# fzaiser/genfer

Hardware: AMD Instinct MI355X
Metric: TaylorPoly mul f64 GMAC/s (higher is better)
Workload: dtype f64

## Files before the change

genfer_amd/csrc/gft_conv_tiled.hip:

```cpp
#include <algorithm>
#include <cstdio>
#include <cstdlib>
#include <cstring>
#include <map>
#include <vector>

#include "gft_kernels.hpp"
#include "gft_peel_layout.hpp"

namespace gft {

namespace {

struct TileSeg {
    unsigned u, a, b;
    unsigned step_begin, step_end;
    int dest;
};

struct RedTile {
    unsigned u, a, b;
    unsigned first, count;
    unsigned slot0;
};

struct TiledArgs {
    unsigned xU, x0, x1, xI;
    unsigned yU, y0, y1, yI;
    unsigned zU, z0, z1, zI;
    unsigned nx8, ny8;
    unsigned nxc, nyc, nb;
    unsigned P1;
    unsigned tsh;
    unsigned slab_axis;
    unsigned slab_lo, slab_hi;
    int accumulate;
    unsigned xcd_remap;
    unsigned cut;
    unsigned lim1;
    size_t zsU, zs0, zs1, zoff;
    const double* xp;
    const double* yp;
    double* z;
    double* ws;
    const TileSeg* segs;
    const unsigned* wg_begin;
    const RedTile* red;
    const unsigned* red_slots;
    const unsigned* guard;
    unsigned guard_epoch;
    unsigned* claim;
    unsigned n_ranges, n_queues;
#ifdef GFT_TILED_DIAG
    unsigned long long* stamps;
#endif
    unsigned char blk1[8], blk2[8];
};

typedef const double __attribute__((address_space(4))) * cptr_t;

#ifndef GFT_TILED_DEFAULT_VARIANT
#define GFT_TILED_DEFAULT_VARIANT 7
#endif
#ifndef GFT_TILED_PEEL_DEFAULT
#define GFT_TILED_PEEL_DEFAULT -1
#endif
#ifndef GFT_TILED_PEEL_LANES_DEFAULT
#define GFT_TILED_PEEL_LANES_DEFAULT -1
#endif
constexpr unsigned PEEL_MIN_EXTENT = 112, PEEL_MIN_INNER = 64;

__device__ inline void loadx(double (&dst)[8], cptr_t p) {
#pragma unroll
    for (int i = 0; i < 8; ++i) dst[i] = p[i];
}

__device__ inline void load8(double (&dst)[8], const double* p) {
#pragma unroll
    for (int i = 0; i < 8; ++i) dst[i] = p[i];
}

__device__ inline void load8_b128(double (&dst)[8], const double* p) {
    const double2* q = reinterpret_cast<const double2*>(__builtin_assume_aligned(p, 16));
#pragma unroll
    for (int i = 0; i < 4; ++i) {
        double2 v = q[i];
        dst[2 * i] = v.x;
        dst[2 * i + 1] = v.y;
    }
}

// ... 351 lines not shown
                double* d = w + ((size_t)c1 * 64 + lane) * 8;
#pragma unroll
                for (int r = 0; r < 8; ++r) d[r] = acc1[r];
            }
            if (has2) {
                double* d = w + ((size_t)c2 * 64 + lane) * 8;
#pragma unroll
                for (int r = 0; r < 8; ++r) d[r] = acc2[r];
            }
        }
    }
#ifdef GFT_TILED_DIAG
    if (A.stamps && tid == 0) A.stamps[3 * (size_t)wg + 1] = __builtin_amdgcn_s_memrealtime();
#endif
    if (!claiming) break;
    }
}

__global__ void __launch_bounds__(256) k_conv_reduce(TiledArgs A, unsigned n_red) {
    const unsigned ti = blockIdx.x, c = blockIdx.y;
    if (ti >= n_red) return;
    if (A.guard && *A.guard == A.guard_epoch) return;
    __shared__ double part[3][64][8];
    const RedTile rt = A.red[ti];
    const unsigned lane = threadIdx.x & 63u, q = threadIdx.x >> 6;
    const unsigned k0 = (64u >> A.tsh) * rt.a + (lane >> A.tsh), k1 = (rt.b << A.tsh) + (lane & ((1u << A.tsh) - 1u));
    bool lane_in = k0 < A.z0 && k1 < A.z1;
    if (A.slab_axis == 1) lane_in = lane_in && k0 >= A.slab_lo && k0 < A.slab_hi;
    else if (A.slab_axis == 2) lane_in = lane_in && k1 >= A.slab_lo && k1 < A.slab_hi;
    double v[8];
#pragma unroll
    for (int r = 0; r < 8; ++r) v[r] = 0.0;
    double* zrow = A.z + A.zoff + (size_t)rt.u * A.zsU + (size_t)k0 * A.zs0 + (size_t)k1 * A.zs1;
    if (lane_in) {
        if (q == 0 && A.accumulate) {
#pragma unroll
            for (int r = 0; r < 8; ++r) {
                unsigned k2 = 8 * c + r;
                if (k2 < A.zI) v[r] = zrow[k2];
            }
        }
        const unsigned lo = (unsigned)((unsigned long long)rt.count * q / 4), hi = (unsigned)((unsigned long long)rt.count * (q + 1) / 4);
        unsigned p = lo;
        if (!A.red_slots) {
            const size_t stride = (size_t)A.nb * 512;
            const double* w = A.ws + (size_t)(rt.slot0 + lo) * stride + ((size_t)c * 64 + lane) * 8;
            for (; p + 4 <= hi; p += 4, w += 4 * stride) {
                double t[4][8];
#pragma unroll
                for (int u = 0; u < 4; ++u)
#pragma unroll
                    for (int r = 0; r < 8; ++r) t[u][r] = w[(size_t)u * stride + r];
#pragma unroll
                for (int u = 0; u < 4; ++u)
#pragma unroll
                    for (int r = 0; r < 8; ++r) v[r] += t[u][r];
            }
        }
        for (; p < hi; ++p) {
            const unsigned slot = A.red_slots ? A.red_slots[rt.first + p] : rt.slot0 + p;
            const double* w = A.ws + (size_t)slot * A.nb * 512 + ((size_t)c * 64 + lane) * 8;
#pragma unroll
            for (int r = 0; r < 8; ++r) v[r] += w[r];
        }
        if (q > 0) {
#pragma unroll
            for (int r = 0; r < 8; ++r) part[q - 1][lane][r] = v[r];
        }
    }
    __syncthreads();
    if (q == 0 && lane_in) {
#pragma unroll
        for (int g = 0; g < 3; ++g)
#pragma unroll
            for (int r = 0; r < 8; ++r) v[r] += part[g][lane][r];
#pragma unroll
        for (int r = 0; r < 8; ++r) {
            unsigned k2 = 8 * c + r;
            if (k2 < A.zI) zrow[k2] = v[r];
        }
    }
}

__global__ void __launch_bounds__(256) k_prep_operands(const double* __restrict__ x, double* __restrict__ xp, size_t x_rows,
                                                       unsigned xlen, unsigned nx8, const double* __restrict__ y,
                                                       double* __restrict__ yp, size_t y_rows, unsigned ylen, unsigned ny8,
                                                       unsigned* flag, unsigned epoch) {
    const size_t tx = x_rows * nx8, ty = yp ? y_rows * ny8 : y_rows * ylen;
    bool bad = false;
    for (size_t i = blockIdx.x * (size_t)blockDim.x + threadIdx.x; i < tx + ty; i += (size_t)gridDim.x * blockDim.x) {
        double v;
        if (i < tx) {
            size_t row = i / nx8;
            unsigned col = (unsigned)(i - row * nx8);
            v = col < xlen ? x[row * xlen + col] : 0.0;
            xp[i] = v;
        } else if (yp) {
            size_t k = i - tx, row = k / ny8;
            unsigned col = (unsigned)(k - row * ny8);
            v = col < ylen ? y[row * ylen + col] : 0.0;
            yp[k] = v;
        } else {
            v = y[i - tx];
        }
        if (!((v - v) == 0.0)) bad = true;
    }
    if (__any(bad) && (threadIdx.x & 63) == 0) atomicMax(flag, epoch);
}

__global__ void __launch_bounds__(256) k_pack_peel(const double* __restrict__ x, const double* __restrict__ y,
                                                   double* __restrict__ w0, double* __restrict__ s1, double* __restrict__ w1,
                                                   unsigned n0, unsigned n1, unsigned nI, unsigned n8) {
    const size_t t0 = (size_t)7 * (n0 / 8) * n1 * n8, ts = (size_t)7 * n0 * n8, t1 = (size_t)7 * (n1 / 8) * n0 * n8;
    for (size_t i = blockIdx.x * (size_t)blockDim.x + threadIdx.x; i < t0 + ts + t1; i += (size_t)gridDim.x * blockDim.x) {
        const double* src;
        double* dst;
        size_t row;
        unsigned col;
        if (i < t0) {
            row = i / n8;
            col = (unsigned)(i - row * n8);
            const unsigned r1 = (unsigned)(row % n1), va = (unsigned)(row / n1), a = va % (n0 / 8), v = va / (n0 / 8);
            src = x + ((size_t)(8 * a + 1 + v) * n1 + r1) * nI;
            dst = w0 + i;
        } else if (i < t0 + ts) {
            const size_t k = i - t0;
            row = k / n8;
            col = (unsigned)(k - row * n8);
            const unsigned j1c = (unsigned)(row % n0), ju = (unsigned)(row / n0);
            src = y + ((size_t)j1c * n1 + ju) * nI;
            dst = s1 + k;
        } else {
            const size_t k = i - t0 - ts;
            row = k / n8;
            col = (unsigned)(k - row * n8);
            const unsigned r = (unsigned)(row % n0), vb = (unsigned)(row / n0), b = vb % (n1 / 8), v = vb / (n1 / 8);
            src = x + ((size_t)r * n1 + 8 * b + 1 + v) * nI;
            dst = w1 + k;
        }
        *dst = col < nI ? src[col] : 0.0;
    }
}

__global__ void __launch_bounds__(256) k_pad_rows(const double* __restrict__ in, double* __restrict__ out, size_t rows,
                                                  unsigned len, unsigned P, unsigned B) {
    const size_t per_p = rows * B, total = per_p * P;
    for (size_t i = blockIdx.x * (size_t)blockDim.x + threadIdx.x; i < total; i += (size_t)gridDim.x * blockDim.x) {
        const unsigned p = (unsigned)(i / per_p);
        const size_t rem = i - (size_t)p * per_p, row = rem / B;
        const unsigned col = p * B + (unsigned)(rem - row * B);
        out[i] = col < len ? in[row * len + col] : 0.0;
    }
}
__global__ void __launch_bounds__(256) k_fold_rows(const double* __restrict__ zt, double* __restrict__ z, size_t rows,
                                                   size_t row_lo, size_t row_hi, unsigned Pz, unsigned B, unsigned zI,
                                                   int accumulate, const unsigned* guard, unsigned epoch) {
    if (guard && *guard == epoch) return;
    const unsigned RI = 2 * B - 1;
    size_t total = (row_hi - row_lo) * zI;
    for (size_t i = blockIdx.x * (size_t)blockDim.x + threadIdx.x; i < total; i += (size_t)gridDim.x * blockDim.x) {
        size_t row = row_lo + i / zI;
        unsigned k = (unsigned)(i % zI), p = k / B, r = k - p * B;
        double v = p < Pz ? zt[((size_t)p * rows + row) * RI + r] : 0.0;
        if (p > 0 && p - 1 < Pz && r + 1 < B) v += zt[((size_t)(p - 1) * rows + row) * RI + B + r];
        double* dst = z + row * zI + k;
        *dst = accumulate ? *dst + v : v;
    }
}


struct Variant {
    bool fast;
    bool b128;
    bool xcd;
    bool compact;
    bool peel;
    unsigned other;
};
static_assert((GFT_TILED_DEFAULT_VARIANT & 3) == 3, "only the pipelined b128 kernel (VAR 3) is instantiated for every NW");
Variant decode_variant(int variant, bool compact_operands) {
    if (variant < 0) variant = GFT_TILED_DEFAULT_VARIANT;
    Variant V = {bool(variant & 1), bool(variant & 2), bool(variant & 4), bool(variant & 8), bool(variant & 128),
                 unsigned(variant & ~(1 | 2 | 4 | 8 | 128))};
    if (compact_operands && V.fast && V.b128) V = {true, true, V.xcd, true, false, 0};
    else if (compact_operands) V.fast = V.b128 = false;
    return V;
}
int pick_var(const Variant& V, unsigned NW) {
    if (V.peel) return 131;
    if (V.compact) return 11;
    if (V.fast == V.b128 && !V.other) return V.fast ? 3 : 0;
    return (NW == 8 && V.fast && !V.b128 && !V.xcd) ? 1 + (int)V.other : -1;
}

struct PlanKey {
    unsigned v[19];
    bool operator<(const PlanKey& o) const { return std::memcmp(v, o.v, sizeof(v)) < 0; }
};

struct Plan {
    TiledArgs base;
    unsigned n_wg = 0, n_red = 0, n_slots = 0, NW = 0;
    unsigned n_resident = 0;
    unsigned n_segs = 0;
    bool all_slabs = false;
    size_t lds_bytes = 0;
    void* d_tables = nullptr;
};

struct TableArena {
    char* dev = nullptr;
    char* host = nullptr;
    size_t bytes = 0, head = 0;
    bool tried = false;
    bool ensure() {
        if (dev) return true;
        if (tried) return false;
        tried = true;
        const size_t n = 32u << 20;
        if (hipMalloc((void**)&dev, n) != hipSuccess) { dev = nullptr; (void)hipGetLastError(); return false; }
        if (hipHostMalloc((void**)&host, n, hipHostMallocDefault) != hipSuccess) {
            (void)hipFree(dev);
            dev = nullptr;
            (void)hipGetLastError();
// ... 345 lines not shown
    else GFT_LAUNCH((k_conv_tiled<NW, VAR | 256, TSH>), dim3(grid), dim3(NW * 64), P.lds_bytes, st, T);
}
template <int NW, int VAR>
void launch_main_nw(hipStream_t st, const Plan& P, const TiledArgs& T, unsigned grid) {
    if (T.tsh == 3) launch_main_t<NW, VAR, 3>(st, P, T, grid);
    else launch_main_t<NW, VAR, 0>(st, P, T, grid);
}
template <int VAR>
void launch_main(hipStream_t st, const Plan& P, const TiledArgs& T, unsigned grid) {
    switch (P.NW) {
        case 1: launch_main_nw<1, VAR>(st, P, T, grid); break;
        case 2: launch_main_nw<2, VAR>(st, P, T, grid); break;
        case 4: launch_main_nw<4, VAR>(st, P, T, grid); break;
        default: launch_main_nw<8, VAR>(st, P, T, grid); break;
    }
}

}

void tiled_pad_rows_f64(hipStream_t st, const double* in, double* out, size_t rows, unsigned len, unsigned P, unsigned B) {
    size_t tot = rows * P * B;
    if (!tot) return;
    GFT_LAUNCH(k_pad_rows, dim3((unsigned)std::min<size_t>((tot + 255) / 256, 4096)), dim3(256), 0, st, in, out, rows,
                       len, P, B);
}
void tiled_fold_rows_f64(hipStream_t st, const double* zt, double* z, size_t rows, size_t row_lo, size_t row_hi, unsigned Pz,
                         unsigned B, unsigned zI, int accumulate, const unsigned* guard, unsigned epoch) {
    size_t tot = (row_hi - row_lo) * zI;
    if (!tot) return;
    GFT_LAUNCH(k_fold_rows, dim3((unsigned)std::min<size_t>((tot + 255) / 256, 4096)), dim3(256), 0, st, zt, z, rows,
                       row_lo, row_hi, Pz, B, zI, accumulate, guard, epoch);
}

void tiled_set_lane_tile(int tsh) { tiled_force_tsh() = tsh; }
void tiled_set_slots(int n) { tiled_slots_cap() = n; }
void tiled_set_taper(int pct) { tiled_taper_pct() = pct < 0 ? GFT_TILED_TAPER_DEFAULT : std::min(pct, 90); }

namespace {

int& tiled_peel_mode() {
    static int v = GFT_TILED_PEEL_DEFAULT;
    return v;
}
int& tiled_peel_lanes_mode() {
    static int v = GFT_TILED_PEEL_LANES_DEFAULT;
    return v;
}

const Plan* cached_plan(const ConvArgs& a, const Variant& V, const PeelSpec& ps, hipStream_t st) {
    PlanKey key;
    std::memset(&key, 0, sizeof(key));
    if (a.nd < 2 || a.nd > 4) return nullptr;
    key.v[0] = (unsigned)a.nd | ((unsigned)a.slab_axis << 8) | ((unsigned)tiled_force_tsh() << 16) | ((unsigned)tiled_taper_pct() << 24);
    for (int i = 0; i < a.nd; ++i) {
        key.v[1 + i] = a.xs[i];
        key.v[5 + i] = a.ys[i];
        key.v[9 + i] = a.zs[i];
    }
    key.v[13] = a.slab_lo;
    key.v[14] = a.slab_hi;
    key.v[15] = (unsigned)a.accumulate;
    key.v[16] = (unsigned)(a.j0_min | (a.j0_excl << 8) | (a.j0_desc << 16));
    key.v[17] = V.b128;
    key.v[18] = ps.role | (ps.cut << 4) | (ps.lim1 << 8) | (ps.all_slabs << 12);
    auto& cache = plan_cache();
    auto it = cache.find(key);
    if (it == cache.end()) {
        Plan P;
        if (cache.size() >= 1024) reset_plan_cache(st);
        if (!build_plan(a, V, ps, P, st)) return nullptr;
        it = cache.emplace(key, P).first;
    }
    return &it->second;
}

unsigned launch_grid(const Plan& P) {
    if (tiled_slots_cap() < 0) return P.n_wg;
    unsigned g = std::min(P.n_wg, P.n_resident);
    if (tiled_slots_cap() > 0) g = std::min(g, (unsigned)tiled_slots_cap());
    return g;
}
bool plan_claims(const Plan& P) { return launch_grid(P) < P.n_wg; }
constexpr size_t CLAIM_BYTES = 256;
unsigned* claim_words(char* wb, unsigned launch) { return (unsigned*)wb + 8 * launch; }
void zero_claim_words(hipStream_t st, char* wb) {
    enqueue_task([=] { lq_note((hipMemsetAsync)(wb, 0, CLAIM_BYTES, st), nullptr, "hipMemsetAsync"); });
}

#ifdef GFT_TILED_DIAG
constexpr unsigned STAMP_RANGES = 65536;
unsigned long long* stamp_area(unsigned launch, const Plan& first) {
    static unsigned long long* d_stamps = nullptr;
    const char* stamps_min = std::getenv("GFT_TILED_STAMPS_MIN");
    if (!std::getenv("GFT_TILED_STAMPS") || first.n_wg < (stamps_min ? (unsigned)std::atoi(stamps_min) : 1024u)) return nullptr;
    if (!d_stamps && hipMalloc((void**)&d_stamps, 3 * (size_t)3 * STAMP_RANGES * sizeof(unsigned long long)) != hipSuccess) d_stamps = nullptr;
    return d_stamps ? d_stamps + (size_t)launch * 3 * STAMP_RANGES : nullptr;
}
struct StampedLaunch {
    const char* name;
    const unsigned long long* d_stamps;
    unsigned n, grid;
    bool claiming;
};
void dump_stamps(hipStream_t st, const StampedLaunch* ls, unsigned n_launches) {
    if (hipStreamSynchronize(st) != hipSuccess) return;
    FILE* f = std::fopen(std::getenv("GFT_TILED_STAMPS"), "a");
    if (!f) return;
    unsigned long long first_end = 0;
    for (unsigned l = 0; l < n_launches; ++l) {
        const unsigned n = ls[l].n;
        std::vector<unsigned long long> h(3 * (size_t)n);
        if (!ls[l].d_stamps || hipMemcpy(h.data(), ls[l].d_stamps, h.size() * 8, hipMemcpyDeviceToHost) != hipSuccess) continue;
        unsigned long long t0 = ~0ull, t1 = 0, last[8] = {0}, busy[8] = {0};
        unsigned cnt[8] = {0};
        for (unsigned r = 0; r < n; ++r) {
            const unsigned long long b = h[3 * (size_t)r], e = h[3 * (size_t)r + 1];
            const unsigned x = (unsigned)h[3 * (size_t)r + 2] & 7u;
            t0 = std::min(t0, b);
            t1 = std::max(t1, e);
            last[x] = std::max(last[x], e);
            busy[x] += e - b;
            cnt[x]++;
        }
        std::fprintf(f, "launch %s: %u ranges on %u workgroups (%s), %.1f us from first start to last end\n", ls[l].name, n, ls[l].grid,
                     ls[l].claiming ? "claiming" : "one range each", (t1 - t0) / 100.0);
        if (l == 0) first_end = t1;
        else
            std::fprintf(f, "  first range starts %+.1f us, last range ends %+.1f us relative to the last range end of launch %s\n",
                         ((double)t0 - (double)first_end) / 100.0, ((double)t1 - (double)first_end) / 100.0, ls[0].name);
        for (int x = 0; x < 8; ++x)
            std::fprintf(f, "  xcd %d: %5u ranges, range time %10.1f us in all, last range ends %8.1f us before the launch's last\n", x, cnt[x],
                         busy[x] / 100.0, (t1 - last[x]) / 100.0);
    }
    std::fclose(f);
}
#endif

bool launch_plan_main(hipStream_t st, const Plan& P, TiledArgs& T, const Variant& V, unsigned* claim) {
    const unsigned grid = launch_grid(P);
    const bool eighths = V.xcd && P.n_wg % 8 == 0;
    T.n_ranges = P.n_wg;
    if (grid < P.n_wg) {
        if (!claim) return false;
        T.claim = claim;
        T.n_queues = eighths ? 8u : 1u;
        T.xcd_remap = 0;
    } else {
        T.claim = nullptr;
        T.n_queues = 1;
        T.xcd_remap = eighths ? 1u : 0u;
    }
#ifdef GFT_TILED_DIAG
    if (P.n_wg > STAMP_RANGES) T.stamps = nullptr;
#endif
    switch (pick_var(V, P.NW)) {
        case 131: launch_main<131>(st, P, T, grid); break;
        case 11: launch_main<11>(st, P, T, grid); break;
        case 3: launch_main<3>(st, P, T, grid); break;
        case 0: launch_main<0>(st, P, T, grid); break;
        case 1: launch_main_nw<8, 1>(st, P, T, grid); break;
#ifdef GFT_TILED_DIAG
        case 17: launch_main_nw<8, 17>(st, P, T, grid); break;
        case 33: launch_main_nw<8, 33>(st, P, T, grid); break;
        case 49: launch_main_nw<8, 49>(st, P, T, grid); break;
        case 65: launch_main_nw<8, 65>(st, P, T, grid); break;
        case 113: launch_main_nw<8, 113>(st, P, T, grid); break;
#endif
        default: return false;
    }
    return true;
}
void launch_plan_reduce(hipStream_t st, const Plan& P, const TiledArgs& T) {
    if (P.n_red) {
        GFT_LAUNCH(k_conv_reduce, dim3(P.n_red, T.nb), dim3(256), 0, st, T, P.n_red);
    }
}
bool launch_plan(hipStream_t st, const Plan& P, TiledArgs T, const Variant& V, unsigned* claim) {
#ifdef GFT_TILED_DIAG
    T.stamps = stamp_area(0, P);
#endif
    if (!launch_plan_main(st, P, T, V, claim)) return false;
#ifdef GFT_TILED_DIAG
    if (T.stamps) {
        const StampedLaunch l = {"plain", T.stamps, P.n_wg, launch_grid(P), plan_claims(P)};
        dump_stamps(st, &l, 1);
    }
#endif
    launch_plan_reduce(st, P, T);
    return true;
}

struct Operands {
    bool inplace, pack_y;
    size_t o_ws, o_xp, o_yp, end;
};
Operands operand_layout(const TiledArgs& B, size_t n_slots, bool claims, const double* x, const double* y, int operands_slack) {
    auto al = [](size_t v) { return (v + 255) / 256 * 256; };
    const size_t x_rows = (size_t)B.xU * B.x0 * B.x1, y_rows = (size_t)B.yU * B.y0 * B.y1;
    Operands o;
    o.inplace = operands_slack && B.nx8 == B.xI && B.ny8 == B.yI && B.nxc >= B.nb && B.nyc >= B.nb && !((uintptr_t)y & 15) &&
                !((uintptr_t)x & 7);
    o.pack_y = !o.inplace && (B.ny8 != B.yI || ((uintptr_t)y & 15));
    o.o_ws = claims ? CLAIM_BYTES : 0;
    o.o_xp = o.o_ws + al(n_slots * B.nb * 512 * sizeof(double));
    o.o_yp = o.o_xp + al((x_rows * B.nx8 + 8) * sizeof(double));
    o.end = o.o_yp + al(y_rows * B.ny8 * sizeof(double));
    return o;
}
void bind_operands(hipStream_t st, const Operands& o, const double* x, const double* y, char* wb, unsigned* nf_flag,
                   unsigned nf_epoch, TiledArgs& T) {
    T.ws = (double*)(wb + o.o_ws);
    if (o.inplace) {
        T.xp = x;
        T.yp = y;
        T.guard = nullptr;
        T.guard_epoch = 0;
        return;
    }
    const size_t x_rows = (size_t)T.xU * T.x0 * T.x1, y_rows = (size_t)T.yU * T.y0 * T.y1;
    double *xp = (double*)(wb + o.o_xp), *yp = (double*)(wb + o.o_yp);
    const size_t tot = x_rows * T.nx8 + (o.pack_y ? y_rows * T.ny8 : y_rows * T.yI);
    GFT_LAUNCH(k_prep_operands, dim3((unsigned)std::min<size_t>((tot + 255) / 256, 2048)), dim3(256), 0, st, x, xp, x_rows, T.xI,
               T.nx8, y, o.pack_y ? yp : nullptr, y_rows, T.yI, T.ny8, nf_flag, nf_epoch);
    T.xp = xp;
    T.yp = o.pack_y ? yp : y;
    T.guard = nf_flag;
    T.guard_epoch = nf_epoch;
}

bool peel_applies(const ConvArgs& a, const Variant& V) {
    const int mode = tiled_peel_mode();
    if (mode == 0) return false;
    if (a.nd != 3 || a.slab_axis != 0 || a.slab_lo != 0 || a.slab_hi != a.zs[0]) return false;
    if (a.j0_min || a.j0_excl || a.j0_desc) return false;
    for (int i = 0; i < 3; ++i)
        if (a.xs[i] != a.zs[i] || a.ys[i] != a.zs[i]) return false;
    const unsigned n0 = a.zs[0], n1 = a.zs[1];
    if (n0 % 8 || n1 % 8 || n0 < 16 || n1 < 16 || a.zs[2] > 128) return false;
    if (!V.fast || !V.b128 || V.compact || V.peel || V.other) return false;
    TiledArgs T;
    std::memset(&T, 0, sizeof(T));
    T.x0 = T.y0 = T.z0 = n0;
    T.x1 = T.y1 = T.z1 = n1;
    if (pick_lane_tile(T) != 3) return false;
    return mode == 1 || (n0 >= PEEL_MIN_EXTENT && n1 >= PEEL_MIN_EXTENT && a.zs[2] >= PEEL_MIN_INNER);
}

int conv_tiled_peel(hipStream_t st, const double* x, const double* y, double* z, const ConvArgs& a, const Variant& V, void* ws,
                    size_t ws_bytes, size_t* ws_needed, unsigned* nf_flag, unsigned nf_epoch, bool* guarded, bool* forked) {
    const unsigned n0 = a.zs[0], n1 = a.zs[1], nI = a.zs[2];
    ConvArgs l0, l1;
    std::memset(&l0, 0, sizeof(l0));
    l0.nd = 4;
    l0.slab_lo = 0;
    l0.slab_hi = 7;
    l0.accumulate = 1;
    l1 = l0;
    Variant VL = V;
    VL.peel = true;
    const unsigned s0x[4] = {7, 1, n1, nI}, s0y[4] = {7, n0 / 8, n1, nI}, s1x[4] = {7, 1, n0, nI}, s1y[4] = {7, n1 / 8, n0, nI};
    for (int i = 0; i < 4; ++i) {
        l0.xs[i] = s0x[i]; l0.ys[i] = l0.zs[i] = s0y[i];
        l1.xs[i] = s1x[i]; l1.ys[i] = l1.zs[i] = s1y[i];
    }
    const int lanes_mode = tiled_peel_lanes_mode();
    bool can_fork = lanes_mode != 0 && stream_lanes().ok;
    if (can_fork) {
        hipStreamCaptureStatus cs = hipStreamCaptureStatusNone;
        if (hipStreamIsCapturing(st, &cs) != hipSuccess) (void)hipGetLastError();
        if (cs != hipStreamCaptureStatusNone) can_fork = false;
    }
    bool fork = can_fork && lanes_mode > 0;
    PeelSpec pm, p0, p1;
    pm.role = 1; pm.cut = 3;
    p0.role = 2; p0.zsU = (size_t)n1 * nI; p0.zs0 = 8 * p0.zsU; p0.zs1 = nI; p0.zoff = p0.zsU;
    p1.role = 3; p1.lim1 = 1; p1.zsU = nI; p1.zs0 = 8 * (size_t)nI; p1.zs1 = (size_t)n1 * nI; p1.zoff = nI;
    Plan PM, P0, P1;
    for (int attempt = 0;; ++attempt) {
        const unsigned long long gen = plan_generation();
        const Plan* q = cached_plan(a, V, pm, st);
        if (!q) return -1;
        PM = *q;
        for (int pass = 0; pass < 2; ++pass) {
            p0.all_slabs = p1.all_slabs = fork ? 1u : 0u;
            if (!(q = cached_plan(l0, VL, p0, st))) return -1;
            P0 = *q;
            if (!(q = cached_plan(l1, VL, p1, st))) return -1;
            P1 = *q;
            if (fork || !can_fork || !(plan_claims(P0) && plan_claims(P1))) break;
            fork = true;
        }
        if (gen == plan_generation()) break;
        if (attempt) return -1;
    }
    const TiledArgs& B = PM.base;
    if (B.tsh != 3) return -1;
    const bool claims = plan_claims(PM) || plan_claims(P0) || plan_claims(P1);
    Operands o = operand_layout(B, 0, claims, x, y, a.operands_slack);
    const size_t slots[3] = {PM.n_slots, P0.n_segs, P1.n_segs};
    const PeelLayout L = peel_layout_for(slots, n0, n1, B.nx8, claims);
    o.o_ws = L.o_slab[0];
    o.o_xp = L.o_xp;
    o.o_yp = L.o_yp;
    if (ws && ws_bytes < L.need) return -1;
    if (ws_needed) *ws_needed = L.need;
    if (guarded) *guarded = !o.inplace;
    if (!ws) return 1;

    const hipStream_t st0 = fork ? stream_lanes().st[0] : st, st1 = fork ? stream_lanes().st[1] : st;
    if (forked) *forked = fork;

    char* wb = (char*)ws;
    double *w0 = (double*)(wb + L.o_w0), *s1 = (double*)(wb + L.o_s1), *w1 = (double*)(wb + L.o_w1);
    TiledArgs T = B;
    if (claims) zero_claim_words(st, wb + L.o_claim);
    bind_operands(st, o, x, y, wb, nf_flag, nf_epoch, T);
    {
        const size_t tot = L.b_w0 / sizeof(double) + (L.b_s1 / sizeof(double) - 8) + L.b_w1 / sizeof(double);
        GFT_LAUNCH(k_pack_peel, dim3((unsigned)std::min<size_t>((tot + 255) / 256, 4096)), dim3(256), 0, st, x, y, w0, s1, w1, n0, n1,
                   nI, B.nx8);
    }
    if (fork) lanes_fork(st);
    T.z = z;
    TiledArgs T0 = P0.base, T1 = P1.base;
    T0.ws = (double*)(wb + L.o_slab[1]);
    T1.ws = (double*)(wb + L.o_slab[2]);
    T0.z = T1.z = z;
    T0.guard = T1.guard = T.guard;
    T0.guard_epoch = T1.guard_epoch = T.guard_epoch;
    T0.xp = T.yp;
    T0.yp = w0;
    T1.xp = s1;
    T1.yp = w1;
#ifdef GFT_TILED_DIAG
    T.stamps = stamp_area(0, PM);
    T0.stamps = stamp_area(1, PM);
    T1.stamps = stamp_area(2, PM);
#endif
    unsigned *const c = claim_words(wb + L.o_claim, 0), *const c0 = claim_words(wb + L.o_claim, 1), *const c1 = claim_words(wb + L.o_claim, 2);
    if (fork) {
        const bool ok = launch_plan_main(st, PM, T, V, c) && launch_plan_main(st0, P0, T0, VL, c0) && launch_plan_main(st1, P1, T1, VL, c1);
        if (ok) launch_plan_reduce(st, PM, T);
        lanes_join(st);
        if (!ok) return 0;
        launch_plan_reduce(st, P0, T0);
        launch_plan_reduce(st, P1, T1);
    } else {
        if (!launch_plan_main(st, PM, T, V, c)) return 0;
        launch_plan_reduce(st, PM, T);
        if (!launch_plan_main(st, P0, T0, VL, c0)) return 0;
        launch_plan_reduce(st, P0, T0);
        if (!launch_plan_main(st, P1, T1, VL, c1)) return 0;
        launch_plan_reduce(st, P1, T1);
    }
#ifdef GFT_TILED_DIAG
    if (T.stamps) {
        const StampedLaunch ls[3] = {{"M", T.stamps, PM.n_wg, launch_grid(PM), plan_claims(PM)},
                                     {"L0", T0.stamps, P0.n_wg, launch_grid(P0), plan_claims(P0)},
                                     {"L1", T1.stamps, P1.n_wg, launch_grid(P1), plan_claims(P1)}};
        dump_stamps(st, ls, 3);
    }
#endif
    return 1;
}

}

void tiled_set_peel(int mode) { tiled_peel_mode() = mode < 0 ? -1 : (mode ? 1 : 0); }
void tiled_set_peel_lanes(int mode) { tiled_peel_lanes_mode() = mode < 0 ? GFT_TILED_PEEL_LANES_DEFAULT : (mode ? 1 : 0); }

bool conv_tiled_f64(hipStream_t st, const double* x, const double* y, double* z, const ConvArgs& a, void* ws, size_t ws_bytes,
                    size_t* ws_needed, unsigned* nf_flag, unsigned nf_epoch, bool* guarded, bool* peeled, bool* forked) {
    bool compact_operands = false;
    if (a.nd >= 2 && a.nd <= 4) {
        const unsigned nb = (a.zs[a.nd - 1] + 7) / 8;
        compact_operands = (a.xs[a.nd - 1] + 7) / 8 < nb || (a.ys[a.nd - 1] + 7) / 8 < nb;
    }
    const Variant V = decode_variant(a.variant, compact_operands);
    if (peeled) *peeled = false;
    if (forked) *forked = false;
    if (peel_applies(a, V)) {
        const int r = conv_tiled_peel(st, x, y, z, a, V, ws, ws_bytes, ws_needed, nf_flag, nf_epoch, guarded, forked);
        if (r >= 0) {
            if (peeled) *peeled = r == 1;
            return r == 1;
        }
    }
    const Plan* P = cached_plan(a, V, PeelSpec(), st);
    if (!P) return false;
    const bool claims = plan_claims(*P);
    const Operands o = operand_layout(P->base, P->n_slots, claims, x, y, a.operands_slack);
    const size_t need = o.end + 256;
    if (guarded) *guarded = !o.inplace;
    if (ws_needed) *ws_needed = need;
    if (!ws) return true;
    if (ws_bytes < need) return false;
    TiledArgs T = P->base;
    if (claims) zero_claim_words(st, (char*)ws);
    bind_operands(st, o, x, y, (char*)ws, nf_flag, nf_epoch, T);
    T.z = z;
    return launch_plan(st, *P, T, V, claim_words((char*)ws, 0));
}

}
```

genfer_amd/csrc/gft_kernels.hip:

```cpp
#include "gft_kernels.hpp"
#include "gft_kernels_int.hpp"

#include <algorithm>
#include <chrono>
#include <condition_variable>
#include <cstring>
#include <mutex>
#include <stdexcept>
#include <string>
#include <thread>

namespace gft {

unsigned long long g_launches = 0;
unsigned long long g_host_horner_stats[16] = {0};
bool g_host_horner_runs = true;
int g_host_simd = -1;
unsigned long long g_launches_in_place = 0;
unsigned long long g_stream_ops = 0;

namespace {
constexpr uint64_t LQ_SLOTS = 1024;
struct LaunchQueue {
    std::atomic<uint64_t> head{0};
// ... 128 lines not shown
            msg += std::string(" launching ") + (name ? name : "a kernel");
        } else if (g_lq_err_what) {
            msg += std::string(" in queued ") + g_lq_err_what;
        }
        msg += " (issued by the launch thread; results computed since are invalid)";
        g_lq_err_set.store(false, std::memory_order_relaxed);
    }
    throw std::runtime_error(msg);
}

bool lq_enabled() { return g_lq.enabled; }
void lq_configure(int device, bool enabled) {
    g_lq.drain();
    g_lq.device = device;
    g_lq.enabled = enabled;
}
void lq_shutdown() {
    g_lq.shutdown();
    g_lq.report();
    g_lq_err_set.store(false);
}
void lq_report() {
    g_lq.drain();
    g_lq.report();
}
void launch_drain_nothrow() { g_lq.drain(); }
void launch_drain() {
    g_lq.drain();
    lq_raise();
}
LaunchSlot* lq_begin() {
    if (!g_lq.worker.joinable()) g_lq.start();
    const uint64_t t = g_lq.tail.load(std::memory_order_relaxed);
    if (g_lq.trace && t - g_lq.head.load(std::memory_order_acquire) >= LQ_SLOTS) {
        const auto t0 = std::chrono::steady_clock::now();
        while (t - g_lq.head.load(std::memory_order_acquire) >= LQ_SLOTS) __builtin_ia32_pause();
        g_lq.tr_full_ns += LaunchQueue::ns_since(t0);
        g_lq.tr_full_n++;
    }
    while (t - g_lq.head.load(std::memory_order_acquire) >= LQ_SLOTS) __builtin_ia32_pause();
    return &g_lq.slots[t & (LQ_SLOTS - 1)];
}
void lq_commit() {
    g_lq.tail.store(g_lq.tail.load(std::memory_order_relaxed) + 1, std::memory_order_seq_cst);
    if (g_lq.sleeping.load(std::memory_order_seq_cst)) {
        std::lock_guard<std::mutex> lk(g_lq.m);
        g_lq.cv.notify_one();
    }
}

StreamLanes& stream_lanes() {
    static StreamLanes l;
    if (!l.tried) {
        l.tried = true;
        int least = 0, greatest = 0;
        if (hipDeviceGetStreamPriorityRange(&least, &greatest) != hipSuccess) least = 0;
        l.ok = hipStreamCreateWithPriority(&l.st[0], hipStreamNonBlocking, least) == hipSuccess &&
               hipStreamCreateWithPriority(&l.st[1], hipStreamNonBlocking, least) == hipSuccess &&
               hipEventCreateWithFlags(&l.fork, hipEventDisableTiming) == hipSuccess && hipEventCreateWithFlags(&l.join[0], hipEventDisableTiming) == hipSuccess &&
               hipEventCreateWithFlags(&l.join[1], hipEventDisableTiming) == hipSuccess;
        if (!l.ok) (void)hipGetLastError();
    }
    return l;
}
void lanes_fork(hipStream_t st) {
    StreamLanes& L = stream_lanes();
    hipEvent_t ev = L.fork;
    hipStream_t a0 = L.st[0], a1 = L.st[1];
    enqueue_task([=] {
        lq_note((hipEventRecord)(ev, st), nullptr, "hipEventRecord (lanes, fork)");
        lq_note((hipStreamWaitEvent)(a0, ev, 0), nullptr, "hipStreamWaitEvent (lane 0)");
        lq_note((hipStreamWaitEvent)(a1, ev, 0), nullptr, "hipStreamWaitEvent (lane 1)");
    });
}
void lanes_join(hipStream_t st) {
    StreamLanes& L = stream_lanes();
    hipEvent_t e0 = L.join[0], e1 = L.join[1];
    hipStream_t a0 = L.st[0], a1 = L.st[1];
    enqueue_task([=] {
        lq_note((hipEventRecord)(e0, a0), nullptr, "hipEventRecord (lane 0)");
        lq_note((hipEventRecord)(e1, a1), nullptr, "hipEventRecord (lane 1)");
        lq_note((hipStreamWaitEvent)(st, e0, 0), nullptr, "hipStreamWaitEvent (lanes, join)");
        lq_note((hipStreamWaitEvent)(st, e1, 0), nullptr, "hipStreamWaitEvent (lanes, join)");
    });
}


template <class E>
__global__ void __launch_bounds__(256) k_gather(const double* __restrict__ src, size_t src_plane,
                                                double* __restrict__ out, size_t out_plane, GatherArgs a,
                                                size_t total) {
    typedef typename E::V V;
    for (size_t lin = blockIdx.x * (size_t)blockDim.x + threadIdx.x; lin < total;
         lin += (size_t)gridDim.x * blockDim.x) {
        size_t r = lin;
        size_t soff = 0;
        bool valid = true;
        unsigned kaxis = 0;
#pragma unroll 1
        for (int ax = a.out.nd - 1; ax >= 0; --ax) {
            unsigned d = a.out.d[ax];
            unsigned k = (unsigned)(r % d);
            r /= d;
            long long si = (long long)k + a.shift[ax];
            if (si < 0 || si >= (long long)a.src_len[ax]) valid = false;
            soff += (size_t)(si < 0 ? 0 : si) * a.src_stride[ax];
            if (ax == a.tab_axis) kaxis = k;
        }
        if (valid && a.keep && !a.keep[kaxis]) valid = false;
        V v = E::zero();
        if (valid) {
            v = E::ld(src, src_plane, soff);
            switch (a.op) {
                case OP_MUL_S: v = E::mul(v, E::from(a.s)); break;
                case OP_DIV_S: v = E::div(v, E::from(a.s)); break;
                case OP_LMUL_S: v = E::mul(E::from(a.s), v); break;
                case OP_NEG: v = E::neg(v); break;
                case OP_MUL_TAB: v = E::mul(v, E::ld(a.tab, a.tab_plane, kaxis)); break;
                case OP_MUL_TAB_LMUL_S: v = E::mul(E::from(a.s), E::mul(v, E::ld(a.tab, a.tab_plane, kaxis))); break;
                case OP_MUL_POW: {
                    const V mv = a.tab ? E::ld(a.tab, a.tab_plane, 0) : E::from(a.s);
                    V f = E::one();
                    for (unsigned i = 0; i < kaxis; ++i) f = E::mul(f, mv);
                    v = E::mul(v, f);
                    break;
                }
                default: break;
            }
        }
        E::st(out, out_plane, lin, v);
    }
}

struct NoTab {};
template <class TAB>
__global__ void __launch_bounds__(256) k_gather_f64x2(const double* __restrict__ src, double* __restrict__ out,
                                                      GatherArgs a, TAB t, size_t total_pairs) {
    const int last = a.out.nd - 1;
    const unsigned half = a.out.d[last] >> 1;
    for (size_t lin = blockIdx.x * (size_t)blockDim.x + threadIdx.x; lin < total_pairs;
         lin += (size_t)gridDim.x * blockDim.x) {
        size_t r = lin / half;
        unsigned kp = (unsigned)(lin - r * half);
        size_t soff = 2 * (size_t)kp;
        bool valid = true;
        unsigned kaxis = 0;
#pragma unroll 1
        for (int ax = last - 1; ax >= 0; --ax) {
            unsigned d = a.out.d[ax];
            unsigned k = (unsigned)(r % d);
            r /= d;
            long long si = (long long)k + a.shift[ax];
            if (si < 0 || si >= (long long)a.src_len[ax]) valid = false;
            soff += (size_t)(si < 0 ? 0 : si) * a.src_stride[ax];
            if (ax == a.tab_axis) kaxis = k;
        }
        if (valid && a.keep && !a.keep[kaxis]) valid = false;
        double2 v = make_double2(0.0, 0.0);
        if (valid) {
            v = *reinterpret_cast<const double2*>(src + soff);
            switch (a.op) {
                case OP_MUL_S: v.x = v.x * a.s.a; v.y = v.y * a.s.a; break;
                case OP_DIV_S: v.x = v.x / a.s.a; v.y = v.y / a.s.a; break;
                case OP_LMUL_S: v.x = a.s.a * v.x; v.y = a.s.a * v.y; break;
                case OP_NEG: v.x = -v.x; v.y = -v.y; break;
                case OP_MUL_TAB: { double f = a.tab[kaxis]; v.x = v.x * f; v.y = v.y * f; break; }
// ... 1795 lines not shown
```

genfer_amd/csrc/gft_launch.hpp:

```cpp
#pragma once
#include <hip/hip_runtime.h>

#include <atomic>
#include <cstddef>
#include <cstdint>
#include <new>
#include <tuple>
#include <type_traits>
#include <utility>

namespace gft {

extern unsigned long long g_launches;
extern unsigned long long g_stream_ops;

constexpr size_t LQ_SLOT_BYTES = 4096;
extern unsigned long long g_launches_in_place;
struct LaunchSlot {
    void (*run)(void*);
    alignas(16) unsigned char payload[LQ_SLOT_BYTES];
};
bool lq_enabled();
void lq_configure(int device, bool enabled);
void lq_shutdown();
// ... 2 lines not shown
void lq_commit();
void launch_drain();
void launch_drain_nothrow();
void lq_note(hipError_t e, const void* kernel, const char* what);
extern std::atomic<int> g_fail_next_launch;

template <class F>
inline void enqueue(F&& f) {
    typedef typename std::decay<F>::type Fn;
    ++g_stream_ops;
    if (!lq_enabled() || sizeof(Fn) > LQ_SLOT_BYTES) {
        if (lq_enabled()) ++g_launches_in_place;
        launch_drain();
        f();
        return;
    }
    LaunchSlot* s = lq_begin();
    new (s->payload) Fn(std::forward<F>(f));
    s->run = [](void* p) {
        Fn* fn = static_cast<Fn*>(p);
        (*fn)();
        fn->~Fn();
    };
    lq_commit();
}
template <class F>
inline void enqueue_task(F&& f) {
    enqueue(std::forward<F>(f));
}

template <class... KArgs>
struct LaunchFn {
    void (*kernel)(KArgs...);
    dim3 grid, block;
    unsigned lds;
    hipStream_t st;
    std::tuple<typename std::decay<KArgs>::type...> t;
    template <class... Args>
    LaunchFn(void (*k)(KArgs...), dim3 g, dim3 b, unsigned l, hipStream_t s, Args&&... args)
        : kernel(k), grid(g), block(b), lds(l), st(s), t(std::forward<Args>(args)...) {}
    void operator()() {
        std::apply([&](auto&... a) { hipLaunchKernelGGL(kernel, grid, block, lds, st, a...); }, t);
        const hipError_t e = hipGetLastError();
        if (e != hipSuccess) lq_note(e, reinterpret_cast<const void*>(kernel), nullptr);
    }
};
template <class... KArgs, class... Args>
inline void launch(void (*kernel)(KArgs...), dim3 grid, dim3 block, size_t lds, hipStream_t st, Args&&... args) {
    typedef LaunchFn<KArgs...> Fn;
    ++g_launches;
    if (g_fail_next_launch.load(std::memory_order_relaxed) && g_fail_next_launch.exchange(0)) lds = (size_t)1 << 20;
    if (!lq_enabled() || sizeof(Fn) > LQ_SLOT_BYTES) {
        enqueue(Fn(kernel, grid, block, (unsigned)lds, st, std::forward<Args>(args)...));
        return;
    }
    ++g_stream_ops;
    LaunchSlot* s = lq_begin();
    new (s->payload) Fn(kernel, grid, block, (unsigned)lds, st, std::forward<Args>(args)...);
    s->run = [](void* p) {
        Fn* fn = static_cast<Fn*>(p);
        (*fn)();
        fn->~Fn();
    };
    lq_commit();
}

inline size_t grant_dynamic_lds(const void* const* ks, size_t nk, size_t want, size_t plain) {
    for (size_t i = 0; i < nk; ++i)
        if (hipFuncSetAttribute(ks[i], hipFuncAttributeMaxDynamicSharedMemorySize, (int)want) != hipSuccess) {
            (void)hipGetLastError();
            return plain;
        }
    return want;
}

struct StreamLanes {
    hipStream_t st[2] = {nullptr, nullptr};
    hipEvent_t fork = nullptr, join[2] = {nullptr, nullptr};
    bool ok = false, tried = false;
};
StreamLanes& stream_lanes();
void lanes_fork(hipStream_t st);
void lanes_join(hipStream_t st);

}

#define GFT_LAUNCH(...) ::gft::launch(__VA_ARGS__)

#ifndef GFT_LAUNCH_NO_WRAP
#define GFT_DRAINED(fn, ...)                              \
    ([&](auto&&... a_) {                                  \
        ++::gft::g_stream_ops;                            \
        ::gft::launch_drain();                            \
        return (fn)(static_cast<decltype(a_)&&>(a_)...);  \
    }(__VA_ARGS__))
#define hipMemcpyAsync(...) GFT_DRAINED(hipMemcpyAsync, __VA_ARGS__)
#define hipMemsetAsync(...) GFT_DRAINED(hipMemsetAsync, __VA_ARGS__)
#define hipMemsetD32Async(...) GFT_DRAINED(hipMemsetD32Async, __VA_ARGS__)
#define hipMemcpy(...) GFT_DRAINED(hipMemcpy, __VA_ARGS__)
#define hipStreamSynchronize(...) GFT_DRAINED(hipStreamSynchronize, __VA_ARGS__)
#define hipStreamQuery(...) GFT_DRAINED(hipStreamQuery, __VA_ARGS__)
#define hipEventRecord(...) GFT_DRAINED(hipEventRecord, __VA_ARGS__)
#define hipStreamWaitEvent(...) GFT_DRAINED(hipStreamWaitEvent, __VA_ARGS__)
#define hipFree(...) GFT_DRAINED(hipFree, __VA_ARGS__)
#define hipStreamDestroy(...) GFT_DRAINED(hipStreamDestroy, __VA_ARGS__)
#endif
```

Baseline: 32010.

## Fuse operand prep, peel packing and claim zeroing into one head kernel

Replaces the separate k_prep_operands, k_pack_peel launches and the claim-word memset with a single k_conv_head kernel. It uses a precomputed per-segment index job, 32-bit indexing and double2 vector loads and stores. It also joins the two side lanes one at a time, so the first lane's reduce can start before the second lane finishes. This cuts launch count and per-element 64-bit divisions, at the cost of more complex indexing and a 32-bit item limit that falls back when exceeded.

```diff
diff --git a/genfer_amd/csrc/gft_conv_tiled.hip b/genfer_amd/csrc/gft_conv_tiled.hip
--- a/genfer_amd/csrc/gft_conv_tiled.hip
+++ b/genfer_amd/csrc/gft_conv_tiled.hip
@@ -7,6 +7,7 @@
 
 #include "gft_kernels.hpp"
 #include "gft_peel_layout.hpp"
+#include "gft_prep_index.hpp"
 
 namespace gft {
 
@@ -524,64 +525,45 @@
     }
 }
 
-__global__ void __launch_bounds__(256) k_prep_operands(const double* __restrict__ x, double* __restrict__ xp, size_t x_rows,
-                                                       unsigned xlen, unsigned nx8, const double* __restrict__ y,
-                                                       double* __restrict__ yp, size_t y_rows, unsigned ylen, unsigned ny8,
-                                                       unsigned* flag, unsigned epoch) {
-    const size_t tx = x_rows * nx8, ty = yp ? y_rows * ny8 : y_rows * ylen;
+template <unsigned SEG>
+__device__ inline bool head_segment(const PrepJob& J, const double* __restrict__ src_base, double* __restrict__ dst_base) {
+    const unsigned len = J.seg[SEG].len, n8 = J.seg[SEG].n8;
     bool bad = false;
-    for (size_t i = blockIdx.x * (size_t)blockDim.x + threadIdx.x; i < tx + ty; i += (size_t)gridDim.x * blockDim.x) {
-        double v;
-        if (i < tx) {
-            size_t row = i / nx8;
-            unsigned col = (unsigned)(i - row * nx8);
-            v = col < xlen ? x[row * xlen + col] : 0.0;
-            xp[i] = v;
-        } else if (yp) {
-            size_t k = i - tx, row = k / ny8;
-            unsigned col = (unsigned)(k - row * ny8);
-            v = col < ylen ? y[row * ylen + col] : 0.0;
-            yp[k] = v;
+    for (unsigned u = blockIdx.x * blockDim.x + threadIdx.x; u < J.seg[SEG].items; u += gridDim.x * blockDim.x) {
+        const PrepItem it = prep_item(J, SEG, u);
+        if (!it.live) continue;
+        const double* src = src_base + (size_t)it.src_row * len + it.col;
+        double2 v;
+        if (it.col + 1 < len && !((uintptr_t)src & 15)) {
+            v = *reinterpret_cast<const double2*>(src);
         } else {
-            v = y[i - tx];
-        }
-        if (!((v - v) == 0.0)) bad = true;
-    }
+            v.x = it.col < len ? src[0] : 0.0;
+            v.y = it.col + 1 < len ? src[1] : 0.0;
+        }
+        if (SEG <= PREP_Y && (!((v.x - v.x) == 0.0) || !((v.y - v.y) == 0.0))) bad = true;
+        if (dst_base) {
+            double* dst = dst_base + (size_t)it.row * n8 + it.col;
+            if (!((uintptr_t)dst & 15)) {
+                *reinterpret_cast<double2*>(dst) = v;
+            } else {
+                dst[0] = v.x;
+                dst[1] = v.y;
+            }
+        }
+    }
+    return bad;
+}
+__global__ void __launch_bounds__(256) k_conv_head(PrepJob J, const double* __restrict__ x, const double* __restrict__ y,
+                                                   double* __restrict__ xp, double* __restrict__ yp, double* __restrict__ w0,
+                                                   double* __restrict__ s1, double* __restrict__ w1, unsigned* claim, unsigned* flag,
+                                                   unsigned epoch) {
+    if (claim && blockIdx.x == 0 && threadIdx.x < PEEL_CLAIM_BYTES / sizeof(unsigned)) claim[threadIdx.x] = 0;
+    bool bad = head_segment<PREP_X>(J, x, xp);
+    bad |= head_segment<PREP_Y>(J, y, yp);
+    head_segment<PREP_W0>(J, x, w0);
+    head_segment<PREP_S1>(J, y, s1);
+    head_segment<PREP_W1>(J, x, w1);
     if (__any(bad) && (threadIdx.x & 63) == 0) atomicMax(flag, epoch);
-}
-
-__global__ void __launch_bounds__(256) k_pack_peel(const double* __restrict__ x, const double* __restrict__ y,
-                                                   double* __restrict__ w0, double* __restrict__ s1, double* __restrict__ w1,
-                                                   unsigned n0, unsigned n1, unsigned nI, unsigned n8) {
-    const size_t t0 = (size_t)7 * (n0 / 8) * n1 * n8, ts = (size_t)7 * n0 * n8, t1 = (size_t)7 * (n1 / 8) * n0 * n8;
-    for (size_t i = blockIdx.x * (size_t)blockDim.x + threadIdx.x; i < t0 + ts + t1; i += (size_t)gridDim.x * blockDim.x) {
-        const double* src;
-        double* dst;
-        size_t row;
-        unsigned col;
-        if (i < t0) {
-            row = i / n8;
-            col = (unsigned)(i - row * n8);
-            const unsigned r1 = (unsigned)(row % n1), va = (unsigned)(row / n1), a = va % (n0 / 8), v = va / (n0 / 8);
-            src = x + ((size_t)(8 * a + 1 + v) * n1 + r1) * nI;
-            dst = w0 + i;
-        } else if (i < t0 + ts) {
-            const size_t k = i - t0;
-            row = k / n8;
-            col = (unsigned)(k - row * n8);
-            const unsigned j1c = (unsigned)(row % n0), ju = (unsigned)(row / n0);
-            src = y + ((size_t)j1c * n1 + ju) * nI;
-            dst = s1 + k;
-        } else {
-            const size_t k = i - t0 - ts;
-            row = k / n8;
-            col = (unsigned)(k - row * n8);
-            const unsigned r = (unsigned)(row % n0), vb = (unsigned)(row / n0), b = vb % (n1 / 8), v = vb / (n1 / 8);
-            src = x + ((size_t)r * n1 + 8 * b + 1 + v) * nI;
-            dst = w1 + k;
-        }
-        *dst = col < nI ? src[col] : 0.0;
-    }
 }
 
 __global__ void __launch_bounds__(256) k_pad_rows(const double* __restrict__ in, double* __restrict__ out, size_t rows,
@@ -1093,10 +1075,8 @@
 }
 bool plan_claims(const Plan& P) { return launch_grid(P) < P.n_wg; }
 constexpr size_t CLAIM_BYTES = 256;
+static_assert(CLAIM_BYTES == PEEL_CLAIM_BYTES, "k_conv_head zeroes PEEL_CLAIM_BYTES");
 unsigned* claim_words(char* wb, unsigned launch) { return (unsigned*)wb + 8 * launch; }
-void zero_claim_words(hipStream_t st, char* wb) {
-    enqueue_task([=] { lq_note((hipMemsetAsync)(wb, 0, CLAIM_BYTES, st), nullptr, "hipMemsetAsync"); });
-}
 
 #ifdef GFT_TILED_DIAG
 constexpr unsigned STAMP_RANGES = 65536;
@@ -1218,25 +1198,32 @@
     o.end = o.o_yp + al(y_rows * B.ny8 * sizeof(double));
     return o;
 }
-void bind_operands(hipStream_t st, const Operands& o, const double* x, const double* y, char* wb, unsigned* nf_flag,
-                   unsigned nf_epoch, TiledArgs& T) {
+void bind_operands(const Operands& o, const double* x, const double* y, char* wb, unsigned* nf_flag, unsigned nf_epoch, TiledArgs& T) {
     T.ws = (double*)(wb + o.o_ws);
-    if (o.inplace) {
-        T.xp = x;
-        T.yp = y;
-        T.guard = nullptr;
-        T.guard_epoch = 0;
-        return;
-    }
-    const size_t x_rows = (size_t)T.xU * T.x0 * T.x1, y_rows = (size_t)T.yU * T.y0 * T.y1;
-    double *xp = (double*)(wb + o.o_xp), *yp = (double*)(wb + o.o_yp);
-    const size_t tot = x_rows * T.nx8 + (o.pack_y ? y_rows * T.ny8 : y_rows * T.yI);
-    GFT_LAUNCH(k_prep_operands, dim3((unsigned)std::min<size_t>((tot + 255) / 256, 2048)), dim3(256), 0, st, x, xp, x_rows, T.xI,
-               T.nx8, y, o.pack_y ? yp : nullptr, y_rows, T.yI, T.ny8, nf_flag, nf_epoch);
-    T.xp = xp;
-    T.yp = o.pack_y ? yp : y;
-    T.guard = nf_flag;
-    T.guard_epoch = nf_epoch;
+    T.xp = o.inplace ? x : (const double*)(wb + o.o_xp);
+    T.yp = o.pack_y ? (const double*)(wb + o.o_yp) : y;
+    T.guard = o.inplace ? nullptr : nf_flag;
+    T.guard_epoch = o.inplace ? 0 : nf_epoch;
+}
+struct PeelGather {
+    double *w0, *s1, *w1;
+    unsigned n0, n1, nI;
+};
+bool launch_head(hipStream_t st, const Operands& o, const double* x, const double* y, char* wb, const TiledArgs& T, unsigned* nf_flag,
+                 unsigned* claim, const PeelGather* g) {
+    if (o.inplace && !g) {
+        if (claim) enqueue_task([=] { lq_note((hipMemsetAsync)(claim, 0, CLAIM_BYTES, st), nullptr, "hipMemsetAsync"); });
+        return true;
+    }
+    const size_t x_rows = o.inplace ? 0 : (size_t)T.xU * T.x0 * T.x1, y_rows = (size_t)T.yU * T.y0 * T.y1;
+    PrepJob J;
+    if (!prep_job(J, x_rows, T.xI, T.nx8, y_rows, T.yI, T.ny8, g != nullptr, g ? g->n0 : 0, g ? g->n1 : 0, g ? g->nI : 0, g ? T.nx8 : 0))
+        return false;
+    double* const none = nullptr;
+    GFT_LAUNCH(k_conv_head, dim3(std::min((J.items + 255) / 256, 2048u)), dim3(256), 0, st, J, x, y, o.inplace ? none : (double*)(wb + o.o_xp),
+               o.pack_y ? (double*)(wb + o.o_yp) : none, g ? g->w0 : none, g ? g->s1 : none, g ? g->w1 : none, claim,
+               o.inplace ? (unsigned*)nullptr : nf_flag, T.guard_epoch);
+    return true;
 }
 
 bool peel_applies(const ConvArgs& a, const Variant& V) {
@@ -1324,13 +1311,9 @@
     char* wb = (char*)ws;
     double *w0 = (double*)(wb + L.o_w0), *s1 = (double*)(wb + L.o_s1), *w1 = (double*)(wb + L.o_w1);
     TiledArgs T = B;
-    if (claims) zero_claim_words(st, wb + L.o_claim);
-    bind_operands(st, o, x, y, wb, nf_flag, nf_epoch, T);
-    {
-        const size_t tot = L.b_w0 / sizeof(double) + (L.b_s1 / sizeof(double) - 8) + L.b_w1 / sizeof(double);
-        GFT_LAUNCH(k_pack_peel, dim3((unsigned)std::min<size_t>((tot + 255) / 256, 4096)), dim3(256), 0, st, x, y, w0, s1, w1, n0, n1,
-                   nI, B.nx8);
-    }
+    bind_operands(o, x, y, wb, nf_flag, nf_epoch, T);
+    const PeelGather gather = {w0, s1, w1, n0, n1, nI};
+    if (!launch_head(st, o, x, y, wb, T, nf_flag, claims ? claim_words(wb + L.o_claim, 0) : nullptr, &gather)) return 0;
     if (fork) lanes_fork(st);
     T.z = z;
     TiledArgs T0 = P0.base, T1 = P1.base;
@@ -1352,9 +1335,10 @@
     if (fork) {
         const bool ok = launch_plan_main(st, PM, T, V, c) && launch_plan_main(st0, P0, T0, VL, c0) && launch_plan_main(st1, P1, T1, VL, c1);
         if (ok) launch_plan_reduce(st, PM, T);
-        lanes_join(st);
+        lanes_join_one(st, 0);
+        if (ok) launch_plan_reduce(st, P0, T0);
+        lanes_join_one(st, 1);
         if (!ok) return 0;
-        launch_plan_reduce(st, P0, T0);
         launch_plan_reduce(st, P1, T1);
     } else {
         if (!launch_plan_main(st, PM, T, V, c)) return 0;
@@ -1407,8 +1391,8 @@
     if (!ws) return true;
     if (ws_bytes < need) return false;
     TiledArgs T = P->base;
-    if (claims) zero_claim_words(st, (char*)ws);
-    bind_operands(st, o, x, y, (char*)ws, nf_flag, nf_epoch, T);
+    bind_operands(o, x, y, (char*)ws, nf_flag, nf_epoch, T);
+    if (!launch_head(st, o, x, y, (char*)ws, T, nf_flag, claims ? claim_words((char*)ws, 0) : nullptr, nullptr)) return false;
     T.z = z;
     return launch_plan(st, *P, T, V, claim_words((char*)ws, 0));
 }
diff --git a/genfer_amd/csrc/gft_kernels.hip b/genfer_amd/csrc/gft_kernels.hip
--- a/genfer_amd/csrc/gft_kernels.hip
+++ b/genfer_amd/csrc/gft_kernels.hip
@@ -234,6 +234,15 @@
         lq_note((hipEventRecord)(e1, a1), nullptr, "hipEventRecord (lane 1)");
         lq_note((hipStreamWaitEvent)(st, e0, 0), nullptr, "hipStreamWaitEvent (lanes, join)");
         lq_note((hipStreamWaitEvent)(st, e1, 0), nullptr, "hipStreamWaitEvent (lanes, join)");
+    });
+}
+void lanes_join_one(hipStream_t st, int lane) {
+    StreamLanes& L = stream_lanes();
+    hipEvent_t e = L.join[lane];
+    hipStream_t a = L.st[lane];
+    enqueue_task([=] {
+        lq_note((hipEventRecord)(e, a), nullptr, "hipEventRecord (one lane)");
+        lq_note((hipStreamWaitEvent)(st, e, 0), nullptr, "hipStreamWaitEvent (one lane, join)");
     });
 }
 
diff --git a/genfer_amd/csrc/gft_launch.hpp b/genfer_amd/csrc/gft_launch.hpp
--- a/genfer_amd/csrc/gft_launch.hpp
+++ b/genfer_amd/csrc/gft_launch.hpp
@@ -108,6 +108,7 @@
 StreamLanes& stream_lanes();
 void lanes_fork(hipStream_t st);
 void lanes_join(hipStream_t st);
+void lanes_join_one(hipStream_t st, int lane);
 
 }
 
diff --git a/genfer_amd/csrc/gft_prep_index.hpp b/genfer_amd/csrc/gft_prep_index.hpp
--- /dev/null
+++ b/genfer_amd/csrc/gft_prep_index.hpp
@@ -0,0 +1,86 @@
+#pragma once
+#include <cstddef>
+
+#ifdef __HIPCC__
+#define GFT_PREP_HD __host__ __device__
+#else
+#define GFT_PREP_HD
+#endif
+
+namespace gft {
+
+enum : unsigned { PREP_X = 0, PREP_Y = 1, PREP_W0 = 2, PREP_S1 = 3, PREP_W1 = 4, PREP_SEGS = 5 };
+
+struct PrepSeg {
+    unsigned rows;
+    unsigned len, n8;
+    unsigned lsh;
+    unsigned ppr;
+    unsigned items;
+};
+
+struct PrepJob {
+    PrepSeg seg[PREP_SEGS];
+    unsigned n0, n1;
+    unsigned items;
+};
+
+struct PrepItem {
+    bool live;
+    unsigned row;
+    unsigned src_row;
+    unsigned col;
+};
+
+inline bool prep_add_seg(PrepJob& J, unsigned s, size_t rows, unsigned len, unsigned n8) {
+    PrepSeg& S = J.seg[s];
+    S.len = len;
+    S.n8 = n8;
+    S.lsh = 2;
+    while (S.lsh < 6 && (2u << S.lsh) < n8) S.lsh++;
+    S.ppr = n8 ? (n8 + (2u << S.lsh) - 1) / (2u << S.lsh) : 0;
+    const unsigned long long items = (unsigned long long)rows * S.ppr << S.lsh;
+    if (rows > 0x7fffffffu || J.items + items > 0x7fffffffu) return false;
+    S.rows = (unsigned)rows;
+    S.items = (unsigned)items;
+    J.items += S.items;
+    return true;
+}
+
+inline bool prep_job(PrepJob& J, size_t x_rows, unsigned xlen, unsigned nx8, size_t y_rows, unsigned ylen, unsigned ny8, bool peel,
+                     unsigned n0, unsigned n1, unsigned nI, unsigned n8) {
+    J = PrepJob();
+    J.n0 = n0;
+    J.n1 = n1;
+    if (peel && (unsigned long long)n0 * n1 > 0x7fffffffu) return false;
+    bool ok = prep_add_seg(J, PREP_X, x_rows, xlen, nx8);
+    ok = ok && prep_add_seg(J, PREP_Y, x_rows ? y_rows : 0, ylen, ny8);
+    ok = ok && prep_add_seg(J, PREP_W0, peel ? (size_t)7 * (n0 / 8) * n1 : 0, nI, n8);
+    ok = ok && prep_add_seg(J, PREP_S1, peel ? (size_t)7 * n0 : 0, nI, n8);
+    ok = ok && prep_add_seg(J, PREP_W1, peel ? (size_t)7 * (n1 / 8) * n0 : 0, nI, n8);
+    return ok;
+}
+
+GFT_PREP_HD inline PrepItem prep_item(const PrepJob& J, unsigned s, unsigned u) {
+    PrepItem it;
+    const PrepSeg& S = J.seg[s];
+    const unsigned piece = u >> S.lsh, lane = u & ((1u << S.lsh) - 1);
+    const unsigned row = S.ppr == 1 ? piece : piece / S.ppr, part = piece - row * S.ppr;
+    it.row = row;
+    it.col = 2 * ((part << S.lsh) + lane);
+    it.live = it.col < S.n8;
+    it.src_row = row;
+    if (s == PREP_W0) {
+        const unsigned va = row / J.n1, r1 = row - va * J.n1, v = va / (J.n0 / 8), a = va - v * (J.n0 / 8);
+        it.src_row = (8 * a + 1 + v) * J.n1 + r1;
+    } else if (s == PREP_S1) {
+        const unsigned ju = row / J.n0, j1c = row - ju * J.n0;
+        it.src_row = j1c * J.n1 + ju;
+    } else if (s == PREP_W1) {
+        const unsigned vb = row / J.n0, r = row - vb * J.n0, v = vb / (J.n1 / 8), b = vb - v * (J.n1 / 8);
+        it.src_row = r * J.n1 + 8 * b + 1 + v;
+    }
+    return it;
+}
+
+}
```

Result: no change. 32120 (median of 6 runs) (+0.3%).
